# roryclear/clearcam

Hardware: AMD Instinct MI355X
Metric: yolov9c_640x640_frames_per_sec (higher is better)
Workload: dtype f16; 1 GPU; YOLOv9-C f16h batch=64 640x640 frames (letterbox 640) per GPU, uint8 BGR frames resident in HBM, seeded synthetic weights, full detect path (letterbox+convs+decode+top300+NMS); batch_per_gpu=64, parallelism=one camera batch per GPU x1, no collective, batches_in_flight=3

## Files before the change

clearcam_amd/csrc/conv_mfma.hip:

```cpp
#include <algorithm>
#include <vector>
#include "conv_select.h"
#include "conv_tile.h"

namespace cc {

template <class T, int BM, int BN, int WM, bool SIMPLE, int CPRW, int NS, int NTH = 2 * BM>
__global__ __launch_bounds__(NTH) void conv_mfma_kernel(const ConvP p, const ConvAux a) {
  constexpr int NT = NTH, WN = NT / 64 / WM;
  constexpr int MI = BM / WM / 16, NJ = BN / WN / 16;
  constexpr int E = 16 / (int)sizeof(T);
  constexpr int BK = CPRW * E;
  constexpr int RPP = NT / CPRW;
  constexpr int XR = BM / RPP;
  constexpr int WR = BN / RPP;
  constexpr int LPS = XR + WR;
  constexpr int STAGE = (BM + BN) * CPRW;
  static_assert(BN % RPP == 0, "BN too small for this row width");
  static_assert(NS * STAGE * 16 >= BM * BN * 2, "epilogue tile must fit in the stages");
  static_assert(MI >= 1 && NJ >= 1, "bad wave layout");
  static_assert((NS - 2) * LPS < 64, "vmcnt is a 6-bit counter");
  extern __shared__ __attribute__((aligned(16))) uint4 lds[];

  const int tid = threadIdx.x, lane = tid & 63, wave = tid >> 6;
// ... 116 lines not shown

  int issued = 0;
#pragma unroll
  for (int s = 0; s < NS - 1; ++s)
    if (s < nkt) { if (s > 0) advance_k(); issue_loads(s); ++issued; }
  int st_c = 0, st_i = NS - 1;
  for (int kt = 0; kt < nkt; ++kt) {
    const int ahead = issued - kt - 1;
    if (NS > 5 && ahead >= 4) wait_vmcnt<4 * LPS>();
    else if (NS > 4 && ahead >= 3) wait_vmcnt<3 * LPS>();
    else if (NS > 3 && ahead >= 2) wait_vmcnt<2 * LPS>();
    else if (NS > 2 && ahead >= 1) wait_vmcnt<LPS>();
    else wait_vmcnt<0>();
    __syncthreads();
    if (issued < nkt) { advance_k(); issue_loads(st_i); ++issued; if (++st_i == NS) st_i = 0; }
    const uint4* ldsX = lds + st_c * STAGE;
    const uint4* ldsW = ldsX + BM * CPRW;
    if (++st_c == NS) st_c = 0;
#pragma unroll
    for (int h = 0; h < CPRW / 4; ++h) {
      uint4 xf[MI], wf[NJ];
#pragma unroll
      for (int i = 0; i < MI; ++i) { const int row = wm0 + i * 16 + fr; xf[i] = ldsX[row * CPRW + ((h * 4 + fg) ^ swz<CPRW>(row))]; }
#pragma unroll
      for (int j = 0; j < NJ; ++j) { const int row = wn0 + j * 16 + fr; wf[j] = ldsW[row * CPRW + ((h * 4 + fg) ^ swz<CPRW>(row))]; }
#pragma unroll
      for (int j = 0; j < NJ; ++j)
#pragma unroll
        for (int i = 0; i < MI; ++i) Mma<T>::run(wf[j], xf[i], acc[j][i]);
    }
  }

  conv_epilogue<T, BM, BN, WM, MI, NJ, NT>(p, acc, n0, lds, [&](int row) { const int m = m0 + row; return m < M ? (long)m : -1L; });
}

template <class T, int TS>
__global__ __launch_bounds__(256, (TS == 256 ? 1 : 2)) void conv_big_kernel(const ConvP p, const ConvAux a) {
  constexpr int BM = TS, BN = TS, NT = 256, WM = 2, WN = 2, MI = BM / WM / 16, NJ = BN / WN / 16;
  constexpr int NF = MI + NJ, MF = MI * NJ, MPG = MF / NF;
  constexpr int E = 8, CPRW = 8, BK = 64, RPP = NT / CPRW, XR = BM / RPP, WR = BN / RPP;
  constexpr int STAGE = (BM + BN) * CPRW;
  static_assert(XR + WR == NF && MF % NF == 0 && NF % 2 == 0, "one DMA piece and MF/NF MFMAs per fragment read");
  static_assert(sizeof(T) == 2, "16-bit storage only");
  extern __shared__ __attribute__((aligned(16))) uint4 lds[];
  const int tid = threadIdx.x, lane = tid & 63, wave = tid >> 6;
  const int M = p.B * p.Ho * p.Wo, hw = p.Ho * p.Wo;
  const unsigned lds_base = lds_addr(lds);
  int wg;
  {
    const int nwg = gridDim.x, bid = blockIdx.x;
    const int q = nwg >> 3, r = nwg & 7, xcd = bid & 7, idx = bid >> 3;
    wg = (xcd < r ? xcd * (q + 1) : r * (q + 1) + (xcd - r) * q) + idx;
  }
  const int mt_ = wg / a.nt;
  const int m0 = mt_ * BM, n0 = (wg - mt_ * a.nt) * BN;

  const int ppos = tid % CPRW, prow = tid / CPRW;
  const int chunk = ppos ^ swz<CPRW>(prow);
  const char* rowp[XR]; unsigned vmask[XR];
  const char* cur[XR]; unsigned inc[XR];
#pragma unroll
  for (int i = 0; i < XR; ++i) {
    const int m = m0 + prow + RPP * i;
    if (a.is1x1) {
      rowp[i] = reinterpret_cast<const char*>(p.s0.ptr) + ((size_t)m * p.s0.cstride + p.s0.coff) * sizeof(T);
      vmask[i] = m < M ? 1u : 0u;
    } else {
      const int mm = m < M ? m : 0;
      const int b = fdiv(mm, hw, a.inv_hw), rem = mm - b * hw, ho = fdiv(rem, p.Wo, a.inv_wo), wo = rem - ho * p.Wo;
      const int h0 = ho * p.stride - p.pad, w0 = wo * p.stride - p.pad;
      unsigned hm = 0, wmk = 0;
#pragma unroll
      for (int r = 0; r < 3; ++r) {
        hm |= (unsigned)(r < p.ks && (unsigned)(h0 + r) < (unsigned)p.Hin) << r;
        wmk |= (unsigned)(r < p.ks && (unsigned)(w0 + r) < (unsigned)p.Win) << r;
      }
      const unsigned vm = ((hm & 1u) ? wmk : 0u) | ((hm & 2u) ? wmk << p.ks : 0u) | ((hm & 4u) ? wmk << (2 * p.ks) : 0u);
      vmask[i] = m < M ? vm : 0u;
      rowp[i] = reinterpret_cast<const char*>(p.s0.ptr) +
                ((((long)b * p.s0.H + h0) * p.s0.W + w0) * (long)p.s0.cstride + p.s0.coff) * (long)sizeof(T);
    }
  }
  const char* wcur[WR]; unsigned winc[WR];
#pragma unroll
  for (int i = 0; i < WR; ++i) {
    const int n = n0 + prow + RPP * i;
    const bool ok = n < p.Cout;
    wcur[i] = ok ? reinterpret_cast<const char*>(p.w) + ((size_t)n * p.Kw + chunk * E) * sizeof(T) : reinterpret_cast<const char*>(&g_zero16);
    winc[i] = ok ? (unsigned)(BK * sizeof(T)) : 0u;
  }
  int k0 = chunk * E, kc, kr, ks_, vt;
  if (k0 < p.Cin) { kc = k0; kr = 0; ks_ = 0; vt = 0; }
  else { vt = k0 / p.Cin; kc = k0 - vt * p.Cin; const int tap = vt >> p.split; kr = tap / p.ks; ks_ = tap - kr * p.ks; }
  auto retarget = [&]() {
    const bool kok = kr < p.ks;
    const int tbit = kr * p.ks + ks_;
    const long delta = ((long)(kr * p.s0.W + ks_) * p.s0.cstride + kc) * (long)sizeof(T);
#pragma unroll
    for (int i = 0; i < XR; ++i) {
      const bool ok = kok && ((vmask[i] >> tbit) & 1u);
      cur[i] = ok ? rowp[i] + delta : reinterpret_cast<const char*>(&g_zero16);
      inc[i] = ok ? (unsigned)(BK * sizeof(T)) : 0u;
    }
  };
  retarget();
  auto advance_k = [&]() {
    k0 += BK; kc += BK;
#pragma unroll
    for (int i = 0; i < WR; ++i) wcur[i] += winc[i];
    if (kc >= p.Cin) {
      do { kc -= p.Cin; ++vt; if (next_filter_tap(vt, p.split)) { if (++ks_ == p.ks) { ks_ = 0; ++kr; } } } while (kc >= p.Cin);
      retarget();
    } else {
#pragma unroll
      for (int i = 0; i < XR; ++i) cur[i] += inc[i];
    }
  };
  auto issue_piece = [&](int stage, int q) {
    const unsigned sbase = __builtin_amdgcn_readfirstlane(lds_base + (unsigned)(stage * STAGE + wave * 64) * 16u);
    if (q < XR) glds16_m0(cur[q], sbase + q * (NT * 16u));
    else glds16_m0(wcur[q - XR], sbase + (BM * CPRW + (q - XR) * NT) * 16u);
  };

  const int wm0 = (wave % WM) * (BM / WM), wn0 = (wave / WM) * (BN / WN);
  const int fr = lane & 15, fg = lane >> 4;
  const int nkt = (p.Ktot + BK - 1) / BK;
  f32x4 acc[NJ][MI];
#pragma unroll
  for (int j = 0; j < NJ; ++j)
#pragma unroll
    for (int i = 0; i < MI; ++i) acc[j][i] = f32x4{0.f, 0.f, 0.f, 0.f};

  uint4 f0[NF], f1[NF];
  auto frag = [&](int stage, int h, int q) -> uint4 {
    const int row = (q < MI ? wm0 + q * 16 : BM + wn0 + (q - MI) * 16) + fr;
    const int srow = q < MI ? row : row - BM;
    return lds[stage * STAGE + row * CPRW + ((h * 4 + fg) ^ swz<CPRW>(srow))];
  };

#pragma unroll
  for (int q = 0; q < XR + WR; ++q) issue_piece(0, q);
  if (nkt > 1) {
    advance_k();
#pragma unroll
    for (int q = 0; q < XR + WR; ++q) issue_piece(1, q);
    wait_vmcnt<XR + WR>();
  } else {
    wait_vmcnt<0>();
  }
  __syncthreads();
#pragma unroll
  for (int q = 0; q < NF; ++q) f0[q] = frag(0, 0, q);

  auto step = [&](int kt, auto more_tag, auto more2_tag) {
    constexpr bool MORE = decltype(more_tag)::value, MORE2 = decltype(more2_tag)::value;
    const int st = kt & 1;
#pragma unroll
    for (int g = 0; g < NF; ++g) {
      f1[g] = frag(st, 1, g);
#pragma unroll
      for (int u = 0; u < MPG; ++u) { const int e = g * MPG + u, j = e / MI, i = e % MI; Mma<T>::run(f0[MI + j], f0[i], acc[j][i]); }
      __builtin_amdgcn_sched_barrier(0);
    }
#pragma unroll
    for (int g = 0; g < NF / 2; ++g) {
#pragma unroll
      for (int u = 0; u < MPG; ++u) { const int e = g * MPG + u, j = e / MI, i = e % MI; Mma<T>::run(f1[MI + j], f1[i], acc[j][i]); }
      __builtin_amdgcn_sched_barrier(0);
    }
    if constexpr (MORE) {
      wait_vmcnt<0>();
      __syncthreads();
      if constexpr (MORE2) advance_k();
    }
#pragma unroll
    for (int g = NF / 2; g < NF; ++g) {
      const int q = 2 * (g - NF / 2);
      if constexpr (MORE2) { issue_piece(st, q); issue_piece(st, q + 1); }
      if constexpr (MORE) { f0[q] = frag(st ^ 1, 0, q); f0[q + 1] = frag(st ^ 1, 0, q + 1); }
#pragma unroll
      for (int u = 0; u < MPG; ++u) { const int e = g * MPG + u, j = e / MI, i = e % MI; Mma<T>::run(f1[MI + j], f1[i], acc[j][i]); }
      __builtin_amdgcn_sched_barrier(0);
    }
  };
  int kt = 0;
  for (; kt + 2 < nkt; ++kt) step(kt, std::true_type{}, std::true_type{});
  if (kt + 1 < nkt) { step(kt, std::true_type{}, std::false_type{}); ++kt; }
  step(kt, std::false_type{}, std::false_type{});
  conv_epilogue<T, BM, BN, WM, MI, NJ, NT>(p, acc, n0, lds, [&](int row) { const int m = m0 + row; return m < M ? (long)m : -1L; });
}

struct WsAux { float inv_tiles, inv_tx; int tiles, tx, total; };

template <class T, int CIN, int COUT>
__global__ __launch_bounds__(256) void conv3x3_ws_kernel(const ConvP p, const WsAux a) {
  constexpr int BM = 128, WM = 2, WN = 2, MI = 4, NJ = COUT / WN / 16;
  constexpr int E = 8, CPRW = CIN / E;
  constexpr int PW = 18, RPP = 256 / CPRW;
  constexpr int XPASS = (180 + RPP - 1) / RPP, PROWS = XPASS * RPP;
  constexpr int XP = PROWS * CPRW;
  constexpr int WROWS = 9 * COUT, WPASS = (WROWS + RPP - 1) / RPP;
  constexpr int WL = WPASS * RPP * CPRW;
  constexpr int ET = BM * COUT * 2 / 16;
  constexpr int HS = CPRW / 4;
  static_assert(sizeof(T) == 2 && (CIN == 32 || CIN == 64) && (COUT == 32 || COUT == 64), "narrow 16-bit layers only");
  extern __shared__ __attribute__((aligned(16))) uint4 lds[];
  uint4* ldsW = lds;
  uint4* ldsE = lds + WL + 2 * XP;
  const int tid = threadIdx.x, lane = tid & 63, wave = tid >> 6;
  const unsigned lds_base = lds_addr(lds);
  const int ppos = tid % CPRW, prow = tid / CPRW;

#pragma unroll
  for (int i = 0; i < WPASS; ++i) {
    const int R = prow + RPP * i;
    const int tap = R / COUT, n = R - tap * COUT;
    const int chunk = ppos ^ swz<CPRW>(R);
    const void* src = (R < WROWS && n < p.Cout) ? static_cast<const void*>(reinterpret_cast<const char*>(p.w) +
                          ((size_t)n * p.Kw + tap * CIN + chunk * E) * sizeof(T)) : static_cast<const void*>(&g_zero16);
    glds16(src, __builtin_amdgcn_readfirstlane(lds_base + (unsigned)((RPP * i) * CPRW + wave * 64) * 16u));
  }

  auto issue_patch = [&](int tile, int buf) {
    const int b = fdiv(tile, a.tiles, a.inv_tiles), trem = tile - b * a.tiles, ty = fdiv(trem, a.tx, a.inv_tx), tx = trem - ty * a.tx;
    const int h0 = ty * 8 - 1, w0 = tx * 16 - 1;
#pragma unroll
    for (int i = 0; i < XPASS; ++i) {
      const int pr = prow + RPP * i;
      const int py = pr / PW, px = pr - py * PW;
      const int ih = h0 + py, iw = w0 + px;
      const bool ok = pr < 180 && (unsigned)ih < (unsigned)p.Hin && (unsigned)iw < (unsigned)p.Win;
      const int chunk = ppos ^ swz<CPRW>(pr);
      const void* src = ok ? static_cast<const void*>(reinterpret_cast<const char*>(p.s0.ptr) +
                                 ((((long)b * p.s0.H + ih) * p.s0.W + iw) * (long)p.s0.cstride + p.s0.coff + chunk * E) * (long)sizeof(T))
                           : static_cast<const void*>(&g_zero16);
      glds16(src, __builtin_amdgcn_readfirstlane(lds_base + (unsigned)(WL + buf * XP + (RPP * i) * CPRW + wave * 64) * 16u));
    }
  };

  const int wm = wave & 1, wn0 = (wave >> 1) * (COUT / WN);
  const int fr = lane & 15, fg = lane >> 4;
  int tile = blockIdx.x, buf = 0;
  if (tile < a.total) issue_patch(tile, 0);
  for (; tile < a.total; tile += gridDim.x, buf ^= 1) {
    wait_vmcnt<0>();
    __syncthreads();
    if (tile + (int)gridDim.x < a.total) issue_patch(tile + gridDim.x, buf ^ 1);
    const uint4* ldsX = lds + WL + buf * XP;
    f32x4 acc[NJ][MI];
#pragma unroll
    for (int j = 0; j < NJ; ++j)
#pragma unroll
      for (int i = 0; i < MI; ++i) acc[j][i] = f32x4{0.f, 0.f, 0.f, 0.f};
#pragma unroll
    for (int tap = 0; tap < 9; ++tap) {
      const int r = tap / 3, sft = tap % 3;
#pragma unroll
      for (int h = 0; h < HS; ++h) {
        uint4 xf[MI], wf[NJ];
#pragma unroll
        for (int i = 0; i < MI; ++i) {
          const int row = (wm * 4 + i + r) * PW + fr + sft;
          xf[i] = ldsX[row * CPRW + ((h * 4 + fg) ^ swz<CPRW>(row))];
        }
#pragma unroll
        for (int j = 0; j < NJ; ++j) {
          const int row = tap * COUT + wn0 + j * 16 + fr;
          wf[j] = ldsW[row * CPRW + ((h * 4 + fg) ^ swz<CPRW>(row))];
        }
#pragma unroll
        for (int j = 0; j < NJ; ++j)
#pragma unroll
          for (int i = 0; i < MI; ++i) Mma<T>::run(wf[j], xf[i], acc[j][i]);
      }
    }
    const int b = fdiv(tile, a.tiles, a.inv_tiles), trem = tile - b * a.tiles, ty = fdiv(trem, a.tx, a.inv_tx), tx = trem - ty * a.tx;
    conv_epilogue<T, BM, COUT, WM, MI, NJ>(p, acc, 0, ldsE, [&](int row) {
      const int ho = ty * 8 + (row >> 4), wo = tx * 16 + (row & 15);
      return (ho < p.Ho && wo < p.Wo) ? ((long)b * p.Ho + ho) * p.Wo + wo : -1L;
    });
  }
}

template <class T> static bool supported_t(const ConvP& p) {
  const int E = 16 / (int)sizeof(T);
  auto src_ok = [&](const Src& s) { return s.C == 0 || (s.C % E == 0 && s.coff % E == 0 && s.cstride % E == 0 && ((uintptr_t)s.ptr & 15) == 0); };
  if (!src_ok(p.s0) || !src_ok(p.s1)) return false;
  if (p.Cin % E || p.Cout % 4 || p.out_coff % 4 || p.out_cstride % 4) return false;
  if (p.res && (p.res_coff % 4 || p.res_cstride % 4)) return false;
  if (p.s0.C + p.s1.C != p.Cin || p.Ktot != p.ks * p.ks * p.Cin * (p.split ? 2 : 1)) return false;
  if (p.split && (sizeof(T) != 2 || p.s0.shift < 0)) return false;
  if (p.Kw < (p.Ktot + 8 * E - 1) / (8 * E) * (8 * E)) return false;
  if ((long)p.B * p.Ho * p.Wo >= (1L << 31) || (long)p.Ho * p.Wo >= (1L << 22)) return false;
  return true;
}

bool conv_mfma_supported(int dt, const ConvP& p) {
  return dt == F32 ? supported_t<float>(p) : supported_t<f16_t>(p);
}

bool conv_persist_ok(const ConvP& p);
bool conv_tile64_legal(const ConvP& p);
void launch_conv_tile64(int dt, const ConvP& p, const ConvChoice& c, hipStream_t stream);
bool conv_wave_legal(const ConvP& p);
void launch_conv_wave(int dt, const ConvP& p, const ConvChoice& c, hipStream_t stream);
bool conv_stream_legal(const ConvP& p);
void launch_conv_stream(int dt, const ConvP& p, const ConvChoice& c, hipStream_t stream);
void launch_conv_phase(int dt, const ConvP& p, const ConvAux& a, const ConvChoice& c, hipStream_t stream);

std::atomic<int> g_stream_override{-1}, g_phase_flags_override{-1}, g_tile64_w_override{-1}, g_stream_flags_override{-1};
std::atomic<int> g_stream_abl{0}, g_tile64_abl{0};

const ConvSwitches& conv_switches() {
  static const ConvSwitches s = [] {
    auto env = [](const char* name, int dflt) { const char* e = getenv(name); return e ? atoi(e) : dflt; };
    ConvSwitches w;
    w.stream = env("CLEARCAM_STREAM", 1);
    w.stream_min_pix = env("CLEARCAM_STREAM_MIN_PIX", 200000);
    w.stream_flags = env("CLEARCAM_STREAM_FLAGS", 10);
    w.ws = env("CLEARCAM_WS", 1);
    w.small_tiles = env("CLEARCAM_SMALL_TILES", 1);
    w.small_pix = env("CLEARCAM_SMALL_PIX", 1);
    w.wave = env("CLEARCAM_WAVE", 1);
    w.tile64 = env("CLEARCAM_TILE64", 1);
    w.tile64_w = env("CLEARCAM_TILE64_W", 0);
    w.big_tile = env("CLEARCAM_BIG_TILE", 1);
    w.phase = env("CLEARCAM_PHASE", 2);
    w.phase_flags = env("CLEARCAM_PHASE_FLAGS", -1);
    return w;
  }();
  return s;
}

static bool known_variant(int v) {
  switch (v) {
    case CONV_AUTO: case CONV_DIRECT: case CONV_GENERIC: case CONV_WS: case CONV_BIG256: case CONV_BIG128: case CONV_PHASE: case CONV_WAVE:
    case CONV_SMALL: case CONV_STREAM: case CONV_TILE64: case CONV_SMALL_32_4: case CONV_SMALL_32_6: case CONV_SMALL_64_3:
    case CONV_PIX64_6: case CONV_PIX64_4: case CONV_PIX32_6: case CONV_PIX32_4: return true;
    default: return false;
  }
}

static ConvChoice generic(int bm, int bn, int wm, int cprw, int ns, bool simple) {
  ConvChoice c;
  c.bm = bm; c.bn = bn; c.wm = wm; c.cprw = cprw; c.ns = ns; c.simple = simple;
  c.nth = bm == 256 ? 512 : 256;
  return c;
}

static bool ws_legal(const ConvP& p) {
  return !p.split && p.ks == 3 && p.stride == 1 && p.pad == 1 && p.s1.C == 0 && p.s0.shift == 0 && (p.Cin == 32 || p.Cin == 64) &&
         p.Cout <= 64 && p.Cout % 8 == 0 && p.Hin == p.Ho && p.Win == p.Wo;
}
static bool ws_applicable(const ConvP& p) {
  if (!conv_switches().ws || !ws_legal(p)) return false;
  const long covered = (long)((p.Ho + 7) / 8 * 8) * ((p.Wo + 15) / 16 * 16);
  if ((long)p.Ho * p.Wo * 5 < covered * 4) return false;
  if (p.Cin == 32 && p.Cout <= 32) return true;
  const long tiles = (long)p.B * (covered / 128);
  return tiles >= 256L * 32;
}
static ConvChoice ws_choice(const ConvP& p) {
  ConvChoice c; c.kernel = ConvKernel::Ws; c.cin = p.Cin; c.cout = p.Cout > 32 ? 64 : 32;
  return c;
}

static bool choose_small(const ConvP& p, int M, bool simple, ConvChoice& c) {
  const int v = p.variant;
  const bool force = v != CONV_AUTO;
  if (!force && !conv_switches().small_tiles) return false;
  const long mt = (M + 127) / 128, b32 = mt * ((p.Cout + 31) / 32), b64 = mt * ((p.Cout + 63) / 64);
  int bn = 0;
  if (b32 <= 512) bn = 32; else if (b64 <= 512) bn = 64;
  if (force && !bn) bn = 64;
  if (!bn) return false;
  bool deep = bn == 32 && b32 <= 256;
  if (v >= CONV_SMALL_32_4 && v <= CONV_SMALL_64_3) { bn = v == CONV_SMALL_64_3 ? 64 : 32; deep = v == CONV_SMALL_32_6; }
  const long n32 = (p.Cout + 31) / 32, t32 = (long)((M + 31) / 32) * n32, t64 = (long)((M + 63) / 64) * n32;
  int pix = 0, st = 4;
  if (v == CONV_AUTO && conv_switches().small_pix) { if (t32 <= 800) { pix = 32; st = p.Ktot >= 4096 ? 6 : 4; } else if (t64 <= 512) pix = 64; }
  if (v == CONV_PIX64_6) { pix = 64; st = 6; } else if (v == CONV_PIX64_4) pix = 64; else if (v == CONV_PIX32_6) { pix = 32; st = 6; } else if (v == CONV_PIX32_4) pix = 32;
  if (pix) c = generic(pix, 32, pix == 32 ? 2 : 4, 8, st, simple);
  else if (deep) c = generic(128, 32, 4, 8, 6, simple);
  else if (bn == 32) c = generic(128, 32, 4, 8, 4, simple);
  else c = generic(128, 64, 2, 8, 3, simple);
  return true;
}

static ConvChoice phase_choice(const ConvP& p, int M, bool simple, bool two) {
  ConvChoice c; c.kernel = ConvKernel::Phase; c.bm = c.bn = 256; c.nth = 512; c.simple = simple; c.two = two;
  const int ov = g_phase_flags_override.load();
  int flags = ov >= 0 ? ov : conv_switches().phase_flags;
  const bool persist_ok = conv_persist_ok(p);
  if (flags < 0) {
    const bool is1x1 = simple && p.ks == 1 && p.stride == 1 && p.pad == 0 && p.Hin == p.Ho && p.Win == p.Wo;
    const long tiles = (long)((M + 255) / 256) * ((p.Cout + 255) / 256);
    flags = ((tiles >= 640 || (is1x1 && tiles > 256)) && persist_ok) ? 512 : 32;
  }
  const size_t xb = (size_t)p.B * p.s0.H * p.s0.W * p.s0.cstride * 2, wbytes = (size_t)p.Cout * p.Kw * 2;
  const bool buf_ok = xb < ((size_t)1 << 32) - 256 && wbytes < ((size_t)1 << 32) - 256;
  c.flags = flags;
  if ((flags & 512) && persist_ok) c.sched = PHASE_PERSIST;
  else if ((flags & 64) && buf_ok && !two) c.sched = PHASE_BUFFER;
  else c.sched = (flags & 32) ? PHASE_ONE_TILE : PHASE_SCHED0;
  return c;
}

bool conv_tile64_takes(int B, int H, int W) {
  const long per_frame = std::min((long)((H + 7) / 8) * ((W + 31) / 32), (long)((H + 15) / 16) * ((W + 15) / 16));
  return conv_switches().tile64 && (long)B * per_frame >= 256 && per_frame * 256 * 4 <= (long)H * W * 5;
}

ConvChoice choose_conv(int dt, const ConvP& p) {
  const int v = p.variant;
  CC_CHECK(known_variant(v), "conv: ConvP::variant names no kernel");
  ConvChoice c;
  if (v == CONV_DIRECT || !conv_mfma_supported(dt, p)) { c.kernel = ConvKernel::Direct; return c; }
  const int M = p.B * p.Ho * p.Wo;
  const bool simple = p.s1.C == 0 && p.s0.shift == 0 && p.ks <= 3;
  if (dt != F32) {
    const int so = g_stream_override.load(), fo = g_stream_flags_override.load();
    const int stream_on = so >= 0 ? so : conv_switches().stream;
    if (v == CONV_STREAM || (v == CONV_AUTO && stream_on && M >= conv_switches().stream_min_pix && conv_stream_legal(p))) {
      c.kernel = ConvKernel::Stream; c.cin = p.Cin; c.cout = p.Cout; c.flags = fo >= 0 ? fo : conv_switches().stream_flags;
      return c;
    }
    if (v == CONV_AUTO && ws_legal(p) && (long)((M + 127) / 128) * ((p.Cout + 31) / 32) <= 512) return ws_choice(p);
    if ((v == CONV_AUTO || v == CONV_SMALL || v >= CONV_SMALL_32_4) && choose_small(p, M, simple, c)) return c;
    if (v == CONV_TILE64 || (v == CONV_AUTO && conv_tile64_legal(p) && conv_tile64_takes(p.B, p.Ho, p.Wo))) {
      const int wo = g_tile64_w_override.load(), forced = wo >= 0 ? wo : conv_switches().tile64_w;
      const long t32 = (long)((p.Ho + 7) / 8) * ((p.Wo + 31) / 32), t16 = (long)((p.Ho + 15) / 16) * ((p.Wo + 15) / 16);
      c.kernel = ConvKernel::Tile64; c.tile64_w = (forced == 16 || (forced != 32 && t16 <= t32)) ? 16 : 32;
      return c;
    }
    const long subtiles = (long)p.B * ((p.Ho + 1) / 2) * ((p.Wo + 15) / 16);
    if (v == CONV_WAVE || (v == CONV_AUTO && conv_switches().wave && conv_wave_legal(p) && p.Cin == 64 && subtiles >= 4096)) {
      c.kernel = ConvKernel::Wave; c.cin = p.Cin; c.cout = p.Cout;
      return c;
    }
    if (v == CONV_WS || (v == CONV_AUTO && ws_applicable(p))) {
      CC_CHECK(ws_legal(p), "weights-stationary 3x3: shape not eligible");
      return ws_choice(p);
    }
  }
  auto padded = [&](int bn) { return (p.Cout + bn - 1) / bn * bn; };
  int bn = 128;
  if (padded(64) < padded(bn)) bn = 64;
  if (padded(32) < padded(bn)) bn = 32;
  if (dt != F32 && p.Cout % 256 == 0) {
    const int big = conv_switches().big_tile, phase = conv_switches().phase;
    const long tiles = (long)((M + 255) / 256) * (p.Cout / 256), rounds = (tiles + 255) / 256;
    const bool fits = p.Ktot >= 1024 && tiles >= 256 && rounds * 256 * 100 <= tiles * 112;
    if ((big > 0 && fits && !p.res && v == CONV_AUTO) || big < 0 || v == CONV_BIG256 || v == CONV_PHASE) bn = 256;
    const long t128 = (long)((M + 127) / 128) * ((p.Cout + 127) / 128);
    const double fill256 = (double)tiles / (double)(rounds * 256), fill128 = (double)t128 / (double)(((t128 + 511) / 512) * 512);
    const bool phase_rule = tiles >= 128 && fill256 * 1.2 >= fill128;
    const bool concat1 = p.s1.C > 0 && p.ks == 1 && p.stride == 1 && p.pad == 0 && p.s0.C % 64 == 0 && p.s1.C % 64 == 0;
    if ((v == CONV_AUTO || (v == CONV_PHASE && concat1)) && (simple || concat1) && p.Cin % 64 == 0 && (phase == 1 || v == CONV_PHASE || (phase != 0 && phase_rule)))
      return phase_choice(p, M, simple, concat1);
  }
  if (v == CONV_BIG128) bn = 128;
  const bool single_barrier = dt != F32 && simple;
  if (bn == 256) {
    if (single_barrier && v == CONV_PHASE) {
      CC_CHECK(p.Cin % 64 == 0 && p.Cout % 256 == 0, "eight-wave 256x256 kernel: Cin must be a multiple of 64 and Cout of 256");
      return phase_choice(p, M, simple, false);
    }
    c = generic(256, 256, 4, 8, 2, simple);
    if (single_barrier) c.kernel = ConvKernel::Big;
    return c;
  }
  if (bn == 128 && single_barrier && (p.Ktot >= 1024 || v == CONV_BIG128)) { c = generic(128, 128, 2, 8, 2, simple); c.kernel = ConvKernel::Big; return c; }
  if (bn == 32) return generic(128, 32, 4, 8, 2, simple);
  if (p.Ktot * (int)dtype_size(dt) <= 512) return generic(128, bn, 2, 4, 2, simple);
  return generic(128, bn, 2, 8, bn == 64 && dt != F32 && p.Ktot >= 2048 ? 3 : 2, simple);
}

template <class T, int BM, int BN, int WM, bool SIMPLE, int CPRW, int NS, int NTH>
static void launch_k(const ConvP& p, const ConvAux& a, hipStream_t stream) {
  constexpr size_t lds = (size_t)NS * (BM + BN) * CPRW * 16;
  const int mtiles = (p.B * p.Ho * p.Wo + BM - 1) / BM;
  ensure_max_lds(conv_mfma_kernel<T, BM, BN, WM, SIMPLE, CPRW, NS, NTH>, lds);
  note_launch(BM == 256 ? "conv_mfma_256" : (BM == 64 ? "conv_mfma_64" : (BM == 32 ? "conv_mfma_32" : "conv_mfma_128")), conv_mfma_kernel<T, BM, BN, WM, SIMPLE, CPRW, NS, NTH>, (long)mtiles * a.nt, NTH, lds);
  hipLaunchKernelGGL((conv_mfma_kernel<T, BM, BN, WM, SIMPLE, CPRW, NS, NTH>), dim3(mtiles * a.nt), dim3(NTH), lds, stream, p, a);
}

template <class T, bool SIMPLE> static void launch_generic(const ConvP& p, const ConvAux& a, const ConvChoice& c, hipStream_t stream) {
#define CC_GENERIC(BM, BN, WM, CPRW, NS, NTH) \
  if (c.bm == BM && c.bn == BN && c.wm == WM && c.cprw == CPRW && c.ns == NS && c.nth == NTH) { launch_k<T, BM, BN, WM, SIMPLE, CPRW, NS, NTH>(p, a, stream); return; }
  CC_GENERIC(128, 128, 2, 8, 2, 256)
  CC_GENERIC(128, 64, 2, 8, 2, 256)
  CC_GENERIC(128, 32, 4, 8, 2, 256)
  CC_GENERIC(128, 128, 2, 4, 2, 256)
  CC_GENERIC(128, 64, 2, 4, 2, 256)
  if constexpr (sizeof(T) == 2) {
    CC_GENERIC(256, 256, 4, 8, 2, 512)
    CC_GENERIC(128, 64, 2, 8, 3, 256)
    CC_GENERIC(128, 32, 4, 8, 4, 256)
    CC_GENERIC(128, 32, 4, 8, 6, 256)
    CC_GENERIC(64, 32, 4, 8, 4, 256)
    CC_GENERIC(64, 32, 4, 8, 6, 256)
    CC_GENERIC(32, 32, 2, 8, 4, 256)
    CC_GENERIC(32, 32, 2, 8, 6, 256)
  }
#undef CC_GENERIC
  CC_CHECK(false, "conv_mfma: no such instantiation of the generic kernel");
}

template <class T, int TS> static void launch_big(const ConvP& p, const ConvAux& a, hipStream_t stream) {
  constexpr size_t lds = (size_t)2 * (2 * TS) * 8 * 16;
  const int M = p.B * p.Ho * p.Wo;
  ensure_max_lds(conv_big_kernel<T, TS>, lds);
  note_launch(TS == 256 ? "conv_big_256" : "conv_big_128", conv_big_kernel<T, TS>, (long)((M + TS - 1) / TS) * a.nt, 256, lds);
  hipLaunchKernelGGL((conv_big_kernel<T, TS>), dim3(((M + TS - 1) / TS) * a.nt), dim3(256), lds, stream, p, a);
}

template <class T, int CIN, int COUT> static void launch_ws(const ConvP& p, hipStream_t stream) {
  constexpr int CPRW = CIN / 8, RPP = 256 / CPRW;
  constexpr int XP = (180 + RPP - 1) / RPP * RPP * CPRW, WL = (9 * COUT + RPP - 1) / RPP * RPP * CPRW;
  constexpr size_t lds = (size_t)(WL + 2 * XP + 128 * COUT * 2 / 16) * 16;
  ensure_max_lds(conv3x3_ws_kernel<T, CIN, COUT>, lds);
  const int cus = cu_count();
  WsAux a{};
  a.tx = (p.Wo + 15) / 16; a.tiles = ((p.Ho + 7) / 8) * a.tx; a.total = p.B * a.tiles;
  a.inv_tiles = 1.0f / (float)a.tiles; a.inv_tx = 1.0f / (float)a.tx;
  const int blocks_per_cu = (int)(160 * 1024 / lds);
  note_launch("conv3x3_ws", conv3x3_ws_kernel<T, CIN, COUT>, (long)a.total, 256, lds, std::min(a.total, cus * std::max(1, blocks_per_cu)));
  hipLaunchKernelGGL((conv3x3_ws_kernel<T, CIN, COUT>), dim3(std::min(a.total, cus * std::max(1, blocks_per_cu))), dim3(256), lds, stream, p, a);
}

template <class T> static void launch_t(const ConvP& p, const ConvAux& a, const ConvChoice& c, hipStream_t stream) {
  if constexpr (sizeof(T) == 2) {
    if (c.kernel == ConvKernel::Ws) {
      if (c.cin == 64) { if (c.cout == 64) launch_ws<T, 64, 64>(p, stream); else launch_ws<T, 64, 32>(p, stream); }
      else { if (c.cout == 64) launch_ws<T, 32, 64>(p, stream); else launch_ws<T, 32, 32>(p, stream); }
      return;
    }
    if (c.kernel == ConvKernel::Big) { if (c.bm == 256) launch_big<T, 256>(p, a, stream); else launch_big<T, 128>(p, a, stream); return; }
  }
  CC_CHECK(c.kernel == ConvKernel::Generic, "conv_mfma: kernel not available for this storage type");
  if (c.simple) launch_generic<T, true>(p, a, c, stream); else launch_generic<T, false>(p, a, c, stream);
}

std::atomic<int> g_route_log{0};
static std::mutex g_route_mutex;
static std::vector<int> g_route_recs;

void route_log_append(const ConvP& p, const ConvChoice& c) {
  const int sym_ho = (p.Hin + 2 * p.pad - p.ks) / p.stride + 1, sym_wo = (p.Win + 2 * p.pad - p.ks) / p.stride + 1;
  const int rec[ROUTE_REC_INTS] = {(int)c.kernel, c.sched, c.bm, c.bn, p.ks, p.stride, (p.Ho > sym_ho || p.Wo > sym_wo) ? 1 : 0, p.act,
                                   p.res ? (p.res_f32 ? 2 : 1) : 0, p.out_f32 ? 1 : 0,
                                   (p.Cout % 8 == 0 && p.out_coff % 8 == 0 && p.out_cstride % 8 == 0) ? 1 : 0,
                                   p.B, p.Hin, p.Win, p.Cin, p.Cout, p.Ho, p.Wo};
  std::lock_guard<std::mutex> lock(g_route_mutex);
  g_route_recs.insert(g_route_recs.end(), rec, rec + ROUTE_REC_INTS);
}

int route_log_take(int* recs, int cap) {
  std::lock_guard<std::mutex> lock(g_route_mutex);
  const int n = (int)(g_route_recs.size() / ROUTE_REC_INTS), take = std::min(n, std::max(cap, 0));
  if (recs && take > 0) std::copy(g_route_recs.begin(), g_route_recs.begin() + (size_t)take * ROUTE_REC_INTS, recs);
  g_route_recs.erase(g_route_recs.begin(), g_route_recs.begin() + (size_t)take * ROUTE_REC_INTS);
  return n;
}

void launch_conv_mfma(int dt, const ConvP& p, hipStream_t stream) { launch_conv_chosen(dt, p, stream, nullptr); }

void launch_conv_chosen(int dt, const ConvP& p, hipStream_t stream, ConvChoice* chosen) {
  const ConvChoice c = choose_conv(dt, p);
  if (chosen) *chosen = c;
  if (g_route_log.load(std::memory_order_relaxed)) route_log_append(p, c);
  ConvAux a{};
  a.nt = (p.Cout + c.bn - 1) / c.bn;
  a.inv_hw = 1.0f / (float)(p.Ho * p.Wo); a.inv_wo = 1.0f / (float)p.Wo;
  a.is1x1 = c.simple && p.ks == 1 && p.stride == 1 && p.pad == 0 && p.Hin == p.Ho && p.Win == p.Wo;
  a.two = c.two;
  switch (c.kernel) {
    case ConvKernel::Direct: launch_conv_direct(dt, p, stream); return;
    case ConvKernel::Stream: launch_conv_stream(dt, p, c, stream); return;
    case ConvKernel::Tile64: launch_conv_tile64(dt, p, c, stream); return;
    case ConvKernel::Wave: launch_conv_wave(dt, p, c, stream); return;
    case ConvKernel::Phase: launch_conv_phase(dt, p, a, c, stream); break;
    default:
      if (dt == F32) launch_t<float>(p, a, c, stream);
      else if (dt == F16) launch_t<f16_t>(p, a, c, stream);
      else launch_t<bf16_t>(p, a, c, stream);
  }
  CC_HIP(hipGetLastError());
}

void launch_conv(int dt, const ConvP& p, hipStream_t stream) {
  if (p.s0.shift < 0) launch_conv_adown(dt, p, stream);
  else launch_conv_mfma(dt, p, stream);
}

}
```

clearcam_amd/csrc/conv_select.h:

```cpp
#pragma once
#include <atomic>
#include "common.h"

namespace cc {

enum ConvVariant : int {
  CONV_AUTO = 0,
  CONV_DIRECT = 1,
  CONV_GENERIC = 2,
  CONV_WS = 4,
  CONV_BIG256 = 5,
  CONV_BIG128 = 6,
  CONV_PHASE = 7,
  CONV_WAVE = 8,
  CONV_SMALL = 9,
  CONV_STREAM = 10,
  CONV_TILE64 = 12,
  CONV_SMALL_32_4 = 91,
  CONV_SMALL_32_6 = 92,
  CONV_SMALL_64_3 = 93,
  CONV_PIX64_6 = 94,
  CONV_PIX64_4 = 95,
  CONV_PIX32_6 = 96,
  CONV_PIX32_4 = 97,
};

enum class ConvKernel : int { Direct, Generic, Big, Phase, Ws, Wave, Tile64, Stream };

enum { PHASE_SCHED0 = 0, PHASE_ONE_TILE = 1, PHASE_BUFFER = 2, PHASE_PERSIST = 3 };

struct ConvChoice {
  ConvKernel kernel = ConvKernel::Generic;
  int bm = 128, bn = 128, wm = 2, cprw = 8, ns = 2, nth = 256;
  bool simple = false;
  int sched = 0;
  bool two = false;
  int flags = 0;
  int tile64_w = 32;
  int cin = 0, cout = 0;
};

ConvChoice choose_conv(int dt, const ConvP& p);

bool conv_tile64_takes(int B, int H, int W);

void launch_conv_chosen(int dt, const ConvP& p, hipStream_t stream, ConvChoice* chosen);

constexpr int ROUTE_REC_INTS = 18;
extern std::atomic<int> g_route_log;
void route_log_append(const ConvP& p, const ConvChoice& c);
int route_log_take(int* recs, int cap);

struct ConvSwitches {
  int stream, stream_min_pix, stream_flags;
  int ws, small_tiles, small_pix, wave;
  int tile64, tile64_w;
  int big_tile, phase, phase_flags;
};
const ConvSwitches& conv_switches();

extern std::atomic<int> g_stream_override, g_phase_flags_override, g_tile64_w_override, g_stream_flags_override;
extern std::atomic<int> g_stream_abl, g_tile64_abl;

}
```

clearcam_amd/csrc/dev_bench.hip:

```cpp
#include <cmath>
#include "conv_select.h"
#include "yolo_plan.h"

using namespace cc;

extern "C" {

int cc_conv2d_nhwc(int dtype, const void* x_dev, int B, int H, int W, int Cin, const float* w_oihw, const float* bias,
                   int Cout, int k, int stride, int groups, int act, void* out_dev, int force_direct, void* stream) {
  CC_API_BEGIN
  CC_CHECK(x_dev && w_oihw && out_dev && groups >= 1 && Cin % groups == 0 && Cout % groups == 0, "bad argument");
  HostTensor w, b;
  w.shape = {Cout, Cin / groups, k, k};
  w.data.assign(w_oihw, w_oihw + (size_t)Cout * (Cin / groups) * k * k);
  if (bias) { b.shape = {Cout}; b.data.assign(bias, bias + Cout); }
  const int split = dtype == F16S;
  dtype = storage_dtype(dtype);
  PackedConv pc = pack_convs(dtype, {&w}, {bias ? &b : nullptr}, {groups}, 0, split);
  ConvP c{};
  c.s0 = Src{x_dev, H, W, Cin, 0, Cin, 0}; c.s1 = Src{x_dev, 1, 1, 0, 0, 0, 0};
  c.B = B; c.Hin = H; c.Win = W; c.Cin = Cin; c.ks = k; c.stride = stride; c.pad = k / 2;
  c.Ho = (H + 2 * c.pad - k) / stride + 1; c.Wo = (W + 2 * c.pad - k) / stride + 1; c.Cout = Cout; c.Ktot = k * k * Cin * (1 + split); c.Kw = pc.kw;
  c.split = pc.split; c.oscale = pc.oscale;
  c.w = pc.w; c.bias = pc.bias; c.out = out_dev; c.out_cstride = Cout; c.out_coff = 0; c.out_f32 = 0; c.res = nullptr; c.act = act;
  c.variant = force_direct;
  launch_conv(dtype, c, (hipStream_t)stream);
  CC_HIP(hipStreamSynchronize((hipStream_t)stream));
  hipFree(pc.w); hipFree(pc.bias);
  CC_API_END
}

int cc_attn_bench(int dtype, int B, int L, int H, int causal, int abl, int iters, float* ms) {
  CC_API_BEGIN
  CC_CHECK(ms && iters > 0 && (dtype == F16 || dtype == BF16) && B > 0 && L > 0 && H > 0, "bad argument");
  const int D = H * 64;
  const size_t nq = (size_t)B * L * 3 * D, no = (size_t)B * L * D;
  std::vector<float> hx(std::min<size_t>(nq, (size_t)1 << 22));
  uint32_t st = 777u;
  for (auto& v : hx) { st = st * 1664525u + 1013904223u; v = ((st >> 8) & 0xffff) / 65536.0f - 0.5f; }
  std::vector<char> h16(hx.size() * 2);
  convert_f32_to(dtype, hx.data(), h16.data(), hx.size());
  char *qkv = nullptr, *ctx = nullptr;
  CC_HIP(hipMalloc((void**)&qkv, nq * 2 + 256)); CC_HIP(hipMalloc((void**)&ctx, no * 2 + 256));
  for (size_t off = 0; off < nq * 2; off += h16.size()) CC_HIP(hipMemcpy(qkv + off, h16.data(), std::min(h16.size(), nq * 2 - off), hipMemcpyHostToDevice));
  AttnP a{}; a.qkv = qkv; a.ctx = ctx; a.B = B; a.L = L; a.H = H; a.D = D; a.causal = causal; a.scale = 0.125f; a.abl = abl;
  hipStream_t s; CC_HIP(hipStreamCreateWithFlags(&s, hipStreamNonBlocking));
  hipEvent_t e0, e1; CC_HIP(hipEventCreate(&e0)); CC_HIP(hipEventCreate(&e1));
  for (int i = 0; i < 3; ++i) launch_attention(dtype, a, s);
  CC_HIP(hipEventRecord(e0, s));
  for (int i = 0; i < iters; ++i) launch_attention(dtype, a, s);
  CC_HIP(hipEventRecord(e1, s));
  CC_HIP(hipStreamSynchronize(s));
  float t = 0; CC_HIP(hipEventElapsedTime(&t, e0, e1));
  *ms = t / iters;
  hipEventDestroy(e0); hipEventDestroy(e1); hipStreamDestroy(s);
  hipFree(qkv); hipFree(ctx);
  CC_API_END
}

int cc_dev_set(const char* key, int value) {
  CC_API_BEGIN
  CC_CHECK(key, "null key");
  if (std::string(key) == "phase_flags") cc::g_phase_flags_override = value;
  else if (std::string(key) == "stream") cc::g_stream_override = value;
  else if (std::string(key) == "stream_abl") cc::g_stream_abl = value;
  else if (std::string(key) == "stream_flags") cc::g_stream_flags_override = value;
  else if (std::string(key) == "tile64_abl") cc::g_tile64_abl = value;
  else if (std::string(key) == "tile64_w") cc::g_tile64_w_override = value;
  else if (std::string(key) == "index_slab_rows") cc::g_index_slab_rows = value;
  else if (std::string(key) == "route_log") cc::g_route_log = value ? 1 : 0;
  else throw cc::Error(-22, std::string("cc_dev_set: unknown key ") + key);
  CC_API_END
}

int cc_conv_bench(int dtype, int B, int H, int W, int Cin, int Cout, int k, int stride, int act, int variant, int iters, float* ms) {
  CC_API_BEGIN
  CC_CHECK(ms && iters > 0 && (dtype == F16 || dtype == BF16 || dtype == F16S), "bad argument");
  const int split = dtype == F16S;
  dtype = storage_dtype(dtype);
  HostTensor w, b;
  w.shape = {Cout, Cin, k, k};
  w.data.resize((size_t)Cout * Cin * k * k);
  uint32_t st = 12345u;
  auto rnd = [&]() { st = st * 1664525u + 1013904223u; return ((st >> 8) & 0xffff) / 65536.0f - 0.5f; };
  const float sc = 2.0f / sqrtf((float)Cin * k * k);
  for (auto& v : w.data) v = rnd() * sc;
  b.shape = {Cout}; b.data.assign(Cout, 0.01f);
  PackedConv pc = pack_convs(dtype, {&w}, {&b}, {1}, 0, split);
  const int pad = k / 2, Ho = (H + 2 * pad - k) / stride + 1, Wo = (W + 2 * pad - k) / stride + 1;
  const size_t nin = (size_t)B * H * W * Cin, nout = (size_t)B * Ho * Wo * Cout;
  std::vector<float> hx(std::min<size_t>(nin, (size_t)1 << 24));
  for (auto& v : hx) v = rnd() * 2.0f;
  std::vector<char> hx16(hx.size() * 2);
  convert_f32_to(dtype, hx.data(), hx16.data(), hx.size());
  char *x = nullptr, *out = nullptr;
  CC_HIP(hipMalloc((void**)&x, nin * 2 + 256)); CC_HIP(hipMalloc((void**)&out, nout * 2 + 256));
  for (size_t off = 0; off < nin * 2; off += hx16.size()) CC_HIP(hipMemcpy(x + off, hx16.data(), std::min(hx16.size(), nin * 2 - off), hipMemcpyHostToDevice));
  ConvP c{};
  c.s0 = Src{x, H, W, Cin, 0, Cin, 0}; c.s1 = Src{x, 1, 1, 0, 0, 0, 0};
  c.B = B; c.Hin = H; c.Win = W; c.Cin = Cin; c.ks = k; c.stride = stride; c.pad = pad; c.Ho = Ho; c.Wo = Wo; c.Cout = Cout;
  c.Ktot = k * k * Cin * (1 + split); c.Kw = pc.kw; c.split = pc.split; c.oscale = pc.oscale; c.w = pc.w; c.bias = pc.bias; c.out = out; c.out_cstride = Cout; c.act = act; c.variant = variant;
  hipStream_t s; CC_HIP(hipStreamCreateWithFlags(&s, hipStreamNonBlocking));
  hipEvent_t e0, e1; CC_HIP(hipEventCreate(&e0)); CC_HIP(hipEventCreate(&e1));
  for (int i = 0; i < 3; ++i) launch_conv(dtype, c, s);
  CC_HIP(hipEventRecord(e0, s));
  for (int i = 0; i < iters; ++i) launch_conv(dtype, c, s);
  CC_HIP(hipEventRecord(e1, s));
  CC_HIP(hipStreamSynchronize(s));
  float t = 0; CC_HIP(hipEventElapsedTime(&t, e0, e1));
  *ms = t / iters;
  if (const char* e = getenv("CLEARCAM_BENCH_DUMP")) {
    unsigned long long v[32] = {};
    (void)e;
    CC_HIP(hipMemcpy(v, out + nout * 2, sizeof(v), hipMemcpyDeviceToHost));
    for (int i = 0; i < 32; ++i) fprintf(stderr, "%llu%c", v[i], (i & 3) == 3 ? '\n' : ' ');
  }
  hipEventDestroy(e0); hipEventDestroy(e1); hipStreamDestroy(s);
  hipFree(x); hipFree(out); hipFree(pc.w); hipFree(pc.bias);
  CC_API_END
}

}
```

Before: 6510 frames/s.

## Add patch-based MFMA kernel for 3x3 stride-2 64-to-128 convolutions

Adds a dedicated persistent kernel for 3x3 stride-2 convolutions with 64 input and 128 output channels. Each tile is an 8x16 output patch: the matching input patch is staged in LDS in even/odd column order with a swizzle and double-buffered across tiles, while every wave keeps its weight slice in registers. The kernel is selected automatically ahead of the weight-stationary and tile64 paths when a tile-count heuristic allows, and an env var or override can force it on or off. This targets the downsampling conv in YOLOv9-C, which previously went through generic kernels, at the cost of high register use and a specialised code path to maintain.

```diff
diff --git a/clearcam_amd/csrc/conv_mfma.hip b/clearcam_amd/csrc/conv_mfma.hip
--- a/clearcam_amd/csrc/conv_mfma.hip
+++ b/clearcam_amd/csrc/conv_mfma.hip
@@ -442,13 +442,15 @@
 bool conv_persist_ok(const ConvP& p);
 bool conv_tile64_legal(const ConvP& p);
 void launch_conv_tile64(int dt, const ConvP& p, const ConvChoice& c, hipStream_t stream);
+bool conv_s2p_legal(const ConvP& p);
+void launch_conv_s2p(int dt, const ConvP& p, hipStream_t stream);
 bool conv_wave_legal(const ConvP& p);
 void launch_conv_wave(int dt, const ConvP& p, const ConvChoice& c, hipStream_t stream);
 bool conv_stream_legal(const ConvP& p);
 void launch_conv_stream(int dt, const ConvP& p, const ConvChoice& c, hipStream_t stream);
 void launch_conv_phase(int dt, const ConvP& p, const ConvAux& a, const ConvChoice& c, hipStream_t stream);
 
-std::atomic<int> g_stream_override{-1}, g_phase_flags_override{-1}, g_tile64_w_override{-1}, g_stream_flags_override{-1};
+std::atomic<int> g_stream_override{-1}, g_phase_flags_override{-1}, g_tile64_w_override{-1}, g_stream_flags_override{-1}, g_s2p_override{-1};
 std::atomic<int> g_stream_abl{0}, g_tile64_abl{0};
 
 const ConvSwitches& conv_switches() {
@@ -464,6 +466,7 @@
     w.wave = env("CLEARCAM_WAVE", 1);
     w.tile64 = env("CLEARCAM_TILE64", 1);
     w.tile64_w = env("CLEARCAM_TILE64_W", 0);
+    w.s2p = env("CLEARCAM_S2P", -1);
     w.big_tile = env("CLEARCAM_BIG_TILE", 1);
     w.phase = env("CLEARCAM_PHASE", 2);
     w.phase_flags = env("CLEARCAM_PHASE_FLAGS", -1);
@@ -475,7 +478,7 @@
 static bool known_variant(int v) {
   switch (v) {
     case CONV_AUTO: case CONV_DIRECT: case CONV_GENERIC: case CONV_WS: case CONV_BIG256: case CONV_BIG128: case CONV_PHASE: case CONV_WAVE:
-    case CONV_SMALL: case CONV_STREAM: case CONV_TILE64: case CONV_SMALL_32_4: case CONV_SMALL_32_6: case CONV_SMALL_64_3:
+    case CONV_SMALL: case CONV_STREAM: case CONV_TILE64: case CONV_S2P: case CONV_SMALL_32_4: case CONV_SMALL_32_6: case CONV_SMALL_64_3:
     case CONV_PIX64_6: case CONV_PIX64_4: case CONV_PIX32_6: case CONV_PIX32_4: return true;
     default: return false;
   }
@@ -551,9 +554,17 @@
   return conv_switches().tile64 && (long)B * per_frame >= 256 && per_frame * 256 * 4 <= (long)H * W * 5;
 }
 
+bool conv_s2p_takes(int B, int Ho, int Wo) {
+  const int ov = g_s2p_override.load(), on = ov >= 0 ? ov : conv_switches().s2p;
+  if (on == 0 || on == 1) return on == 1;
+  const long per_frame = (long)((Ho + 7) / 8) * ((Wo + 15) / 16);
+  return (long)B * per_frame >= 256 && per_frame * 128 * 4 <= (long)Ho * Wo * 5;
+}
+
 ConvChoice choose_conv(int dt, const ConvP& p) {
   const int v = p.variant;
   CC_CHECK(known_variant(v), "conv: ConvP::variant names no kernel");
+  CC_CHECK(v != CONV_S2P || (dt != F32 && conv_s2p_legal(p)), "3x3 stride-2 64 -> 128 patch kernel: shape not eligible");
   ConvChoice c;
   if (v == CONV_DIRECT || !conv_mfma_supported(dt, p)) { c.kernel = ConvKernel::Direct; return c; }
   const int M = p.B * p.Ho * p.Wo;
@@ -563,6 +574,10 @@
     const int stream_on = so >= 0 ? so : conv_switches().stream;
     if (v == CONV_STREAM || (v == CONV_AUTO && stream_on && M >= conv_switches().stream_min_pix && conv_stream_legal(p))) {
       c.kernel = ConvKernel::Stream; c.cin = p.Cin; c.cout = p.Cout; c.flags = fo >= 0 ? fo : conv_switches().stream_flags;
+      return c;
+    }
+    if (v == CONV_S2P || (v == CONV_AUTO && conv_s2p_legal(p) && conv_s2p_takes(p.B, p.Ho, p.Wo))) {
+      c.kernel = ConvKernel::S2p;
       return c;
     }
     if (v == CONV_AUTO && ws_legal(p) && (long)((M + 127) / 128) * ((p.Cout + 31) / 32) <= 512) return ws_choice(p);
@@ -719,6 +734,7 @@
     case ConvKernel::Direct: launch_conv_direct(dt, p, stream); return;
     case ConvKernel::Stream: launch_conv_stream(dt, p, c, stream); return;
     case ConvKernel::Tile64: launch_conv_tile64(dt, p, c, stream); return;
+    case ConvKernel::S2p: launch_conv_s2p(dt, p, stream); return;
     case ConvKernel::Wave: launch_conv_wave(dt, p, c, stream); return;
     case ConvKernel::Phase: launch_conv_phase(dt, p, a, c, stream); break;
     default:
diff --git a/clearcam_amd/csrc/conv_s2p.hip b/clearcam_amd/csrc/conv_s2p.hip
--- /dev/null
+++ b/clearcam_amd/csrc/conv_s2p.hip
@@ -0,0 +1,194 @@
+#include <utility>
+#include "conv_select.h"
+#include "conv_tile.h"
+
+namespace cc {
+
+namespace {
+template <int V> using ICs = std::integral_constant<int, V>;
+template <int... I, class F> __device__ __forceinline__ void sfor_s2p_impl(std::integer_sequence<int, I...>, F&& f) { (f(ICs<I>{}), ...); }
+template <int N, class F> __device__ __forceinline__ void sfor_s2p(F&& f) { sfor_s2p_impl(std::make_integer_sequence<int, N>{}, f); }
+typedef __attribute__((ext_vector_type(4))) unsigned s2p_u32x4;
+}
+
+struct S2pAux { float inv_tiles, inv_tx; int tiles, tx, total; };
+
+struct S2pGeom {
+  static constexpr int TH = 8, TW = 16;
+  static constexpr int PH = 2 * TH + 1, PW = 2 * TW + 1, PR = PH * PW;
+  static constexpr int NEVEN = TW + 1;
+  static constexpr int NPIECE = (PR * 8 + 63) / 64;
+  static constexpr int PPW = (NPIECE + 7) / 8;
+  static constexpr int PATCH_BYTES = NPIECE * 1024;
+  static constexpr int NKS = 18;
+  static constexpr int LDS_BYTES = 2 * PATCH_BYTES;
+  static_assert(LDS_BYTES <= 160 * 1024, "LDS budget");
+  static_assert(PPW * 2 <= NKS, "one piece per wave every second k step");
+};
+
+template <class T>
+__global__ __launch_bounds__(512) void conv_s2p_kernel(const ConvP p, const S2pAux a) {
+  using G = S2pGeom;
+  static_assert(sizeof(T) == 2, "16-bit storage");
+  extern __shared__ __attribute__((aligned(16))) uint4 lds[];
+  const char* ldsb = reinterpret_cast<const char*>(lds);
+  const unsigned lds_base = lds_addr(lds);
+  const int tid = threadIdx.x, lane = tid & 63;
+  const int wave = __builtin_amdgcn_readfirstlane(tid >> 6);
+  const int cg = wave & 3, half = wave >> 2;
+  int fr = lane & 15, fg = lane >> 4;
+
+  int tile0, tile_step, n;
+  {
+    const int nwg = gridDim.x, bid = blockIdx.x, xcd = bid & 7, idx = bid >> 3;
+    const int q = a.total >> 3, r = a.total & 7;
+    const int start = xcd * q + (xcd < r ? xcd : r), tile_end = start + q + (xcd < r ? 1 : 0);
+    tile0 = start + idx; tile_step = nwg >> 3;
+    n = tile0 < tile_end ? (tile_end - tile0 + tile_step - 1) / tile_step : 0;
+  }
+  if (n == 0) return;
+  auto tile_origin = [&](int t, int& b, int& h0, int& w0) {
+    b = fdiv(t, a.tiles, a.inv_tiles);
+    const int trem = t - b * a.tiles, ty = fdiv(trem, a.tx, a.inv_tx);
+    h0 = ty * G::TH; w0 = (trem - ty * a.tx) * G::TW;
+  };
+
+  const char* xbase = reinterpret_cast<const char*>(p.s0.ptr) + (size_t)p.s0.coff * 2;
+  auto issue_piece = [&](int k, int b, int h0, int w0, unsigned buf) {
+    const int pi = wave + 8 * k;
+    if (pi < G::NPIECE) {
+      int ln = lane;
+      asm volatile("" : "+v"(ln));
+      const int q = pi * 8 + (ln >> 3), py = q / G::PW, pos = q - py * G::PW;
+      const int px = pos < G::NEVEN ? 2 * pos : 2 * (pos - G::NEVEN) + 1;
+      const int chunk = (ln & 7) ^ (((q >> 1) & 3) << 1);
+      const int ih = 2 * h0 - 1 + py, iw = 2 * w0 - 1 + px;
+      const bool ok = q < G::PR && (unsigned)ih < (unsigned)p.Hin && (unsigned)iw < (unsigned)p.Win;
+      const long off = ((((long)b * p.s0.H + ih) * p.s0.W + iw) * (long)p.s0.cstride + chunk * 8) * 2;
+      const void* src = ok ? static_cast<const void*>(xbase + off) : static_cast<const void*>(&g_zero16);
+      glds16_m0(src, __builtin_amdgcn_readfirstlane(buf + (unsigned)pi * 1024u));
+    }
+  };
+  {
+    int b, h0, w0; tile_origin(tile0, b, h0, w0);
+#pragma unroll
+    for (int k = 0; k < G::PPW; ++k) issue_piece(k, b, h0, w0, lds_base);
+  }
+
+  const int cb = cg * 32;
+  s2p_u32x4 wreg[2][G::NKS];
+  {
+    const T* W = reinterpret_cast<const T*>(p.w);
+#pragma unroll
+    for (int ct = 0; ct < 2; ++ct) {
+      const int co = cb + (fr >> 2) * 8 + ct * 4 + (fr & 3);
+#pragma unroll
+      for (int ks = 0; ks < G::NKS; ++ks) wreg[ct][ks] = *reinterpret_cast<const s2p_u32x4*>(W + (size_t)co * p.Kw + ks * 32 + fg * 8);
+    }
+  }
+  float bv[8] = {0.f, 0.f, 0.f, 0.f, 0.f, 0.f, 0.f, 0.f};
+  if (p.bias) {
+    const float4 b0 = *reinterpret_cast<const float4*>(p.bias + cb + fg * 8), b1 = *reinterpret_cast<const float4*>(p.bias + cb + fg * 8 + 4);
+    bv[0] = b0.x; bv[1] = b0.y; bv[2] = b0.z; bv[3] = b0.w; bv[4] = b1.x; bv[5] = b1.y; bv[6] = b1.z; bv[7] = b1.w;
+  }
+#pragma unroll
+  for (int ct = 0; ct < 2; ++ct)
+#pragma unroll
+    for (int ks = 0; ks < G::NKS; ++ks) asm volatile("" : "+v"(wreg[ct][ks]));
+#pragma unroll
+  for (int e = 0; e < 8; ++e) asm volatile("" : "+v"(bv[e]));
+  wait_vmcnt<0>();
+
+  const float osc = out_scale(p);
+  T* outp = reinterpret_cast<T*>(p.out) + p.out_coff + cb;
+
+  for (int it = 0; it < n; ++it) {
+    asm volatile("" : "+v"(fr), "+v"(fg));
+    __syncthreads();
+    const int pbase = (it & 1) * G::PATCH_BYTES;
+    const unsigned nbuf = lds_base + (unsigned)((it + 1) & 1) * G::PATCH_BYTES;
+    const bool more = it + 1 < n;
+    int nb = 0, nh0 = 0, nw0 = 0;
+    if (more) tile_origin(tile0 + (it + 1) * tile_step, nb, nh0, nw0);
+
+    f32x4 acc[4][2];
+#pragma unroll
+    for (int r = 0; r < 4; ++r)
+#pragma unroll
+      for (int ct = 0; ct < 2; ++ct) acc[r][ct] = f32x4{0.f, 0.f, 0.f, 0.f};
+    const int q0 = (8 * half) * G::PW + fr;
+    auto pix_addr = [&](int q, int c) { const int v = q * 128 + c * 16; return pbase + (v ^ ((v >> 3) & 0x60)); };
+    uint4 xf[2][4];
+    auto rd = [&](auto ks_c) {
+      constexpr int KS = decltype(ks_c)::value, BUF = KS & 1, TAP = KS >> 1, KH = KS & 1, R = TAP / 3, S = TAP - R * 3;
+      constexpr int POS = S == 1 ? G::NEVEN : (S >> 1);
+#pragma unroll
+      for (int r = 0; r < 4; ++r) xf[BUF][r] = *reinterpret_cast<const uint4*>(ldsb + pix_addr(q0 + (2 * r + R) * G::PW + POS, 4 * KH + fg));
+    };
+    rd(ICs<0>{});
+    sfor_s2p<G::NKS>([&](auto ks_c) {
+      constexpr int KS = decltype(ks_c)::value, CUR = KS & 1;
+      if constexpr ((KS & 1) == 0 && KS / 2 < G::PPW) { if (more) issue_piece(KS / 2, nb, nh0, nw0, nbuf); }
+      if constexpr (KS + 1 < G::NKS) rd(ICs<KS + 1>{});
+      __builtin_amdgcn_sched_barrier(0);
+#pragma unroll
+      for (int r = 0; r < 4; ++r)
+#pragma unroll
+        for (int ct = 0; ct < 2; ++ct) Mma<T>::run(__builtin_bit_cast(uint4, wreg[ct][KS]), xf[CUR][r], acc[r][ct]);
+      __builtin_amdgcn_sched_barrier(0);
+    });
+
+    uint4 ov[4];
+    auto outputs = [&](auto act_tag) {
+      constexpr int ACT = decltype(act_tag)::value;
+#pragma unroll
+      for (int r = 0; r < 4; ++r) {
+        float v[8];
+#pragma unroll
+        for (int e = 0; e < 4; ++e) {
+          v[e] = activate<T, ACT>(__builtin_fmaf(acc[r][0][e], osc, bv[e]));
+          v[4 + e] = activate<T, ACT>(__builtin_fmaf(acc[r][1][e], osc, bv[4 + e]));
+        }
+        ov[r] = make_uint4(pack2<T>(v[0], v[1]), pack2<T>(v[2], v[3]), pack2<T>(v[4], v[5]), pack2<T>(v[6], v[7]));
+      }
+    };
+    if (p.act == 1) outputs(ICs<1>{}); else outputs(ICs<0>{});
+    wait_vmcnt<0>();
+    int b, h0, w0; tile_origin(tile0 + it * tile_step, b, h0, w0);
+    const int wo = w0 + fr;
+#pragma unroll
+    for (int r = 0; r < 4; ++r) {
+      const int ho = h0 + 4 * half + r;
+      if (ho < p.Ho && wo < p.Wo) *reinterpret_cast<uint4*>(outp + (((size_t)b * p.Ho + ho) * p.Wo + wo) * (size_t)p.out_cstride + fg * 8) = ov[r];
+    }
+  }
+}
+
+bool conv_s2p_legal(const ConvP& p) {
+  return !p.split && p.ks == 3 && p.stride == 2 && p.pad == 1 && p.s1.C == 0 && p.s0.shift == 0 && p.Cin == 64 && p.Cout == 128 && p.s0.C == 64 &&
+         p.s0.H == p.Hin && p.s0.W == p.Win && p.Ho == (p.Hin - 1) / 2 + 1 && p.Wo == (p.Win - 1) / 2 + 1 && !p.res && !p.out_f32 && p.act <= 1 && !p.slope &&
+         p.Kw >= 576 && p.Kw % 8 == 0 && p.s0.cstride % 8 == 0 && p.s0.coff % 8 == 0 && p.out_cstride % 8 == 0 && p.out_coff % 8 == 0 &&
+         (((uintptr_t)p.s0.ptr | (uintptr_t)p.w | (uintptr_t)p.out) & 15) == 0 && (!p.bias || ((uintptr_t)p.bias & 15) == 0) &&
+         (long)p.B * ((p.Ho + 7) / 8) * ((p.Wo + 15) / 16) < (1L << 22);
+}
+
+template <class T> static void launch_s2p_t(const ConvP& p, hipStream_t stream) {
+  using G = S2pGeom;
+  constexpr int lds = G::LDS_BYTES;
+  ensure_max_lds(conv_s2p_kernel<T>, lds);
+  const int cus = cu_count();
+  S2pAux a{};
+  a.tx = (p.Wo + G::TW - 1) / G::TW; a.tiles = ((p.Ho + G::TH - 1) / G::TH) * a.tx; a.total = p.B * a.tiles;
+  a.inv_tiles = 1.0f / (float)a.tiles; a.inv_tx = 1.0f / (float)a.tx;
+  const int grid = std::max(8, std::min(cus, a.total) & ~7);
+  note_launch("conv_s2p", conv_s2p_kernel<T>, (long)a.total, 512, lds, grid);
+  hipLaunchKernelGGL((conv_s2p_kernel<T>), dim3(grid), dim3(512), lds, stream, p, a);
+}
+
+void launch_conv_s2p(int dt, const ConvP& p, hipStream_t stream) {
+  CC_CHECK(dt != F32 && conv_s2p_legal(p), "3x3 stride-2 64 -> 128 patch kernel: shape not eligible");
+  if (dt == F16) launch_s2p_t<f16_t>(p, stream); else launch_s2p_t<bf16_t>(p, stream);
+  CC_HIP(hipGetLastError());
+}
+
+}
diff --git a/clearcam_amd/csrc/conv_select.h b/clearcam_amd/csrc/conv_select.h
--- a/clearcam_amd/csrc/conv_select.h
+++ b/clearcam_amd/csrc/conv_select.h
@@ -16,6 +16,7 @@
   CONV_SMALL = 9,
   CONV_STREAM = 10,
   CONV_TILE64 = 12,
+  CONV_S2P = 13,
   CONV_SMALL_32_4 = 91,
   CONV_SMALL_32_6 = 92,
   CONV_SMALL_64_3 = 93,
@@ -25,7 +26,7 @@
   CONV_PIX32_4 = 97,
 };
 
-enum class ConvKernel : int { Direct, Generic, Big, Phase, Ws, Wave, Tile64, Stream };
+enum class ConvKernel : int { Direct, Generic, Big, Phase, Ws, Wave, Tile64, Stream, S2p };
 
 enum { PHASE_SCHED0 = 0, PHASE_ONE_TILE = 1, PHASE_BUFFER = 2, PHASE_PERSIST = 3 };
 
@@ -43,6 +44,7 @@
 ConvChoice choose_conv(int dt, const ConvP& p);
 
 bool conv_tile64_takes(int B, int H, int W);
+bool conv_s2p_takes(int B, int Ho, int Wo);
 
 void launch_conv_chosen(int dt, const ConvP& p, hipStream_t stream, ConvChoice* chosen);
 
@@ -55,11 +57,12 @@
   int stream, stream_min_pix, stream_flags;
   int ws, small_tiles, small_pix, wave;
   int tile64, tile64_w;
+  int s2p;
   int big_tile, phase, phase_flags;
 };
 const ConvSwitches& conv_switches();
 
-extern std::atomic<int> g_stream_override, g_phase_flags_override, g_tile64_w_override, g_stream_flags_override;
+extern std::atomic<int> g_stream_override, g_phase_flags_override, g_tile64_w_override, g_stream_flags_override, g_s2p_override;
 extern std::atomic<int> g_stream_abl, g_tile64_abl;
 
 }
diff --git a/clearcam_amd/csrc/dev_bench.hip b/clearcam_amd/csrc/dev_bench.hip
--- a/clearcam_amd/csrc/dev_bench.hip
+++ b/clearcam_amd/csrc/dev_bench.hip
@@ -67,6 +67,7 @@
   else if (std::string(key) == "stream_flags") cc::g_stream_flags_override = value;
   else if (std::string(key) == "tile64_abl") cc::g_tile64_abl = value;
   else if (std::string(key) == "tile64_w") cc::g_tile64_w_override = value;
+  else if (std::string(key) == "s2p") cc::g_s2p_override = value;
   else if (std::string(key) == "index_slab_rows") cc::g_index_slab_rows = value;
   else if (std::string(key) == "route_log") cc::g_route_log = value ? 1 : 0;
   else throw cc::Error(-22, std::string("cc_dev_set: unknown key ") + key);
```

Result: no change. 6563 frames/s, median of 6 (+0.8%).
